# zer0int/OpenVision

Hardware: AMD Instinct MI355X
Metric: images/sec (node) ViT-L/14@224 fwd+InfoNCE (higher is better)
Workload: dtype bf16; 1 GPU; vit-large-patch14-224: image tower + text tower (T=80) + InfoNCE, per-GPU batch 256, formula weights, bf16 MFMA / fp32 accumulate; fp8_mask=0, global_batch=256, micro_batches=1, parallelism=dp1

## Files before the change

### include/ovhip.h

```cpp
#ifndef OVHIP_H
#define OVHIP_H

#include <stddef.h>
#include <stdint.h>

#ifdef __cplusplus
extern "C" {
#endif

#define OV_ABI_VERSION 2

typedef void* ov_stream_t;
typedef uint16_t ov_bf16;

enum ov_status {
    OV_OK = 0,
    OV_ERR_INVALID = -1,
    OV_ERR_UNSUPPORTED = -2,
    OV_ERR_WORKSPACE = -3,
    OV_ERR_NO_DEVICE = -4,
    OV_ERR_HIP = -1000
};

enum ov_dtype { OV_F32 = 0, OV_BF16 = 1 };
// ... 44 lines not shown
int ov_attention_lse(const ov_bf16* qkv, int64_t ld_qkv, ov_bf16* out, int64_t ld_out, float* lse, int B, int L, int H, int hd, float scale,
                     ov_stream_t stream);
int ov_attention_prefix(const ov_bf16* qkv, int64_t ld_qkv, ov_bf16* out, int64_t ld_out, int B, int L, int H, int hd, float scale,
                        int prefix, ov_stream_t stream);

int ov_im2col_patches(const void* image, int img_dtype, ov_bf16* out, int B, int S, int P, int Kpad,
                      ov_stream_t stream);

int ov_im2col_patches_keep(const void* image, int img_dtype, const int* keep, ov_bf16* out, int B, int S, int P, int K, int Kpad,
                           ov_stream_t stream);
int ov_patch_keep_inverse(const int* keep, int* inv, int B, int K, int G, int* err_flag, ov_stream_t stream);
int ov_patch_keep_assemble(const ov_bf16* y, int64_t ldy, const float* cls, const float* pos, const int* keep, float* x, int B, int K,
                           int G, int D, ov_stream_t stream);
int ov_patch_keep_assemble_backward(const float* dx, const int* inv, int B, int K, int G, int D, float* dpos, float* dcls, ov_bf16* dy,
                                    int64_t lddy, ov_stream_t stream);
int ov_col2im_patches_keep(const ov_bf16* dcols, int64_t ldc, const int* inv, void* dimg, int img_dtype, int B, int S, int P, int K,
                           ov_stream_t stream);

int ov_cls_rows(ov_bf16* x, int64_t ldx, const float* cls, const float* pos0, int B, int L, int D,
                ov_stream_t stream);

int ov_mean_pool(const ov_bf16* x, int64_t ldx, float* out, int B, int L, int D, int first,
                 ov_stream_t stream);

int ov_text_embed(const int64_t* tokens, const ov_bf16* table, const ov_bf16* pos, ov_bf16* x,
                  int64_t ldx, int B, int T, int D, int V, int* err_flag, ov_stream_t stream);

int ov_gather_rows(const ov_bf16* x, int64_t ldx, ov_bf16* out, int64_t ldo, int B, int L, int t, int D,
                   ov_stream_t stream);

int ov_convert(const void* src, int src_dtype, int64_t lds, void* dst, int dst_dtype, int64_t ldd,
               int64_t rows, int cols, ov_stream_t stream);

int ov_l2norm(const void* x, int x_dtype, int64_t ldx, float* y, int64_t ldy, int64_t rows, int E,
              ov_stream_t stream);

int ov_logits(const float* X, const float* Y, float* out, int64_t ldo, int n1, int n2, int E, float scale, const float* scale_dev,
              ov_stream_t stream);

int ov_attention_fp8out(const ov_bf16* qkv, int64_t ld_qkv, unsigned char* out8, int64_t ld_out, int B, int L, int H, int hd,
                        float scale, const float* out_amax, float* out_amax_next , ov_stream_t stream);

int ov_gemm_fp8(const unsigned char* A, int64_t lda, const unsigned char* W, int64_t ldw, const float* rowscale,
                const float* colscale, const float* bias, ov_bf16* C, int64_t ldc, int64_t M, int N, int K, int epilogue,
                const ov_bf16* R, int64_t ldr, ov_stream_t stream);

// ... 268 lines not shown
```

### openvision_amd/_lib.py

```python
from __future__ import annotations

import ctypes as C
import os
import threading

_PKG = os.path.dirname(os.path.abspath(__file__))
LIB_PATH = os.path.join(_PKG, "libovhip.so")
if os.environ.get("OVHIP_LIB"):
    LIB_PATH = os.path.join(_PKG, os.environ["OVHIP_LIB"]) if os.sep not in os.environ["OVHIP_LIB"] else os.environ["OVHIP_LIB"]

OV_F32, OV_BF16 = 0, 1
EPI_BIAS, EPI_GELU_ERF, EPI_GELU_TANH, EPI_RESIDUAL = 0, 1, 2, 3

c_void_p, c_int, c_int64, c_float, c_size_t = C.c_void_p, C.c_int, C.c_int64, C.c_float, C.c_size_t


class TowerCfg(C.Structure):
    _fields_ = [("width", c_int), ("layers", c_int), ("heads", c_int), ("mlp", c_int), ("mlp_pad", c_int),
                ("gelu_tanh", c_int), ("ln_eps", c_float)]


class BlockWeights(C.Structure):
    _fields_ = [(n, c_void_p) for n in ("ln1_w", "ln1_b", "qkv_w", "qkv_b", "out_w", "out_b", "ln2_w", "ln2_b",
                                        "fc_w", "fc_b", "proj_w", "proj_b", "qkv_colsum", "fc_colsum")]
# ... 54 lines not shown
    "ov_gemm_rowparts": (c_int, [c_void_p, c_int64, c_void_p, c_int64, c_void_p, c_void_p, c_int64, c_int64, c_int, c_int, c_void_p, c_int64,
                                 c_void_p, c_void_p]),
    "ov_attention": (c_int, [c_void_p, c_int64, c_void_p, c_int64, c_int, c_int, c_int, c_int, c_float, c_void_p]),
    "ov_attention_prefix": (c_int, [c_void_p, c_int64, c_void_p, c_int64, c_int, c_int, c_int, c_int, c_float, c_int, c_void_p]),
    "ov_attention_prefix_backward_workspace_bytes": (c_size_t, [c_int, c_int, c_int, c_int]),
    "ov_attention_prefix_backward": (c_int, [c_void_p, c_int64, c_void_p, c_int64, c_void_p, c_int64, c_void_p, c_int64, c_int, c_int, c_int,
                                             c_int, c_float, c_int, c_void_p, c_size_t, c_void_p]),
    "ov_softmax_xent_workspace_bytes": (c_size_t, [c_int64]),
    "ov_softmax_xent": (c_int, [c_void_p, c_int64, c_void_p, c_void_p, c_int64, c_int, c_void_p, c_void_p, c_void_p, c_size_t, c_void_p]),
    "ov_softmax_xent_backward": (c_int, [c_void_p, c_int64, c_void_p, c_void_p, c_void_p, c_void_p, c_void_p, c_int64, c_int64, c_int,
                                         c_void_p, c_size_t, c_void_p]),
    "ov_tower_set_prefix": (c_int, [c_void_p, c_int]),
    "ov_block_backward_prefix": (c_int, [c_void_p, c_void_p, c_void_p, c_void_p, c_void_p, c_void_p, c_void_p, c_int, c_int, c_int, c_void_p,
                                         c_size_t, c_void_p]),
    "ov_im2col_patches": (c_int, [c_void_p, c_int, c_void_p, c_int, c_int, c_int, c_int, c_void_p]),
    "ov_im2col_patches_keep": (c_int, [c_void_p, c_int, c_void_p, c_void_p, c_int, c_int, c_int, c_int, c_int, c_void_p]),
    "ov_patch_keep_inverse": (c_int, [c_void_p, c_void_p, c_int, c_int, c_int, c_void_p, c_void_p]),
    "ov_patch_keep_assemble": (c_int, [c_void_p, c_int64, c_void_p, c_void_p, c_void_p, c_void_p, c_int, c_int, c_int, c_int, c_void_p]),
    "ov_patch_keep_assemble_backward": (c_int, [c_void_p, c_void_p, c_int, c_int, c_int, c_int, c_void_p, c_void_p, c_void_p, c_int64,
                                                c_void_p]),
    "ov_col2im_patches_keep": (c_int, [c_void_p, c_int64, c_void_p, c_void_p, c_int, c_int, c_int, c_int, c_int, c_void_p]),
    "ov_cls_rows": (c_int, [c_void_p, c_int64, c_void_p, c_void_p, c_int, c_int, c_int, c_void_p]),
    "ov_mean_pool": (c_int, [c_void_p, c_int64, c_void_p, c_int, c_int, c_int, c_int, c_void_p]),
    "ov_text_embed": (c_int, [c_void_p, c_void_p, c_void_p, c_void_p, c_int64, c_int, c_int, c_int, c_int, c_void_p,
                              c_void_p]),
    "ov_gather_rows": (c_int, [c_void_p, c_int64, c_void_p, c_int64, c_int, c_int, c_int, c_int, c_void_p]),
    "ov_convert": (c_int, [c_void_p, c_int, c_int64, c_void_p, c_int, c_int64, c_int64, c_int, c_void_p]),
    "ov_l2norm": (c_int, [c_void_p, c_int, c_int64, c_void_p, c_int64, c_int64, c_int, c_void_p]),
    "ov_logits": (c_int, [c_void_p, c_void_p, c_void_p, c_int64, c_int, c_int, c_int, c_float, c_void_p, c_void_p]),
    "ov_preprocess_image": (c_int, [c_void_p, c_int, c_int, c_void_p, c_void_p, c_int, c_int, c_void_p, c_void_p, c_int, c_int, c_int,
                                    c_int, c_void_p, c_int, c_int, c_int, c_int, c_void_p, c_void_p, c_void_p, c_int, c_void_p]),
    "ov_class_mean_normalize": (c_int, [c_void_p, c_void_p, c_int, c_int, c_int, c_void_p]),
    "ov_topk": (c_int, [c_void_p, c_int64, c_int, c_int, c_int, c_int, c_void_p, c_void_p, c_void_p]),
    "ov_clip_loss_workspace_bytes": (c_size_t, [c_int, c_int]),
    "ov_clip_loss": (c_int, [c_void_p, c_void_p, c_void_p, c_void_p, c_int, c_int, c_int, c_void_p, c_int, c_void_p,
                             c_void_p, c_void_p, c_size_t, c_void_p]),
    "ov_clip_loss_backward_workspace_bytes": (c_size_t, [c_int, c_int]),
    "ov_clip_loss_multi_workspace_bytes": (c_size_t, [c_int, c_int, c_int]),
    "ov_clip_loss_multi": (c_int, [c_void_p, c_void_p, c_void_p, c_void_p, c_int64, c_int64, c_int, c_int, c_int, c_int, c_void_p, c_int,
                                   c_void_p, c_void_p, c_void_p, c_size_t, c_void_p]),
    "ov_clip_loss_multi_backward_workspace_bytes": (c_size_t, [c_int, c_int, c_int]),
    "ov_clip_loss_multi_backward": (c_int, [c_void_p, c_void_p, c_void_p, c_void_p, c_int64, c_int64, c_int, c_int, c_int, c_int, c_void_p,
                                            c_int, c_void_p, c_void_p, c_void_p, c_void_p, c_void_p, c_void_p, c_int64, c_int64, c_void_p,
                                            c_void_p, c_size_t, c_void_p]),
    "ov_siglip_loss_workspace_bytes": (c_size_t, [c_int, c_int]),
    "ov_siglip_loss": (c_int, [c_void_p, c_void_p, c_int, c_int, c_int, c_void_p, c_void_p, c_int, c_void_p, c_void_p, c_size_t,
# ... 130 lines not shown
```

### openvision_amd/csrc/embed.hip

```cpp
#include "common.h"

namespace {

template <bool IMG_F32>
__device__ __forceinline__ u32x4_t im2col_chunk(const void* __restrict__ img, int b, int py, int px, int ch, int S, int P) {
    const int PP = P * P, K = 3 * PP;
    float v[8];
#pragma unroll
    for (int e = 0; e < 8; ++e) {
        const int k = ch * 8 + e;
        float x = 0.f;
        if (k < K) {
            const int c = k / PP, rem = k - c * PP;
            const int ii = rem / P, jj = rem - ii * P;
            const int64_t src = (((int64_t)b * 3 + c) * S + (py * P + ii)) * S + (px * P + jj);
            x = IMG_F32 ? ((const float*)img)[src] : bf16_bits_to_f32(((const ov_bf16*)img)[src]);
        }
        v[e] = x;
    }
    return u32x4_t{pack_bf16x2(v[0], v[1]), pack_bf16x2(v[2], v[3]), pack_bf16x2(v[4], v[5]), pack_bf16x2(v[6], v[7])};
}

template <bool IMG_F32>
__global__ __launch_bounds__(256) void im2col_kernel(const void* __restrict__ img, ov_bf16* __restrict__ out,
// ... 180 lines not shown
        for (int t = first + wave; t < L; t += 4) {
            const u32x4_t w = *(const u32x4_t*)(p + (int64_t)t * ldx);
#pragma unroll
            for (int e = 0; e < 4; ++e) {
                acc[2 * e] += bf16lo_to_f32(w[e]);
                acc[2 * e + 1] += bf16hi_to_f32(w[e]);
            }
        }
    }
#pragma unroll
    for (int e = 0; e < 8; ++e) red[wave][lane][e] = acc[e];
    __syncthreads();
    if (wave == 0 && ch * 8 < D) {
        const float inv = 1.0f / (float)(L - first);
        float o[8];
#pragma unroll
        for (int e = 0; e < 8; ++e) o[e] = (red[0][lane][e] + red[1][lane][e] + red[2][lane][e] + red[3][lane][e]) * inv;
        float4* q = (float4*)(out + (int64_t)b * D + ch * 8);
        q[0] = make_float4(o[0], o[1], o[2], o[3]);
        q[1] = make_float4(o[4], o[5], o[6], o[7]);
    }
}

__global__ __launch_bounds__(256) void text_embed_kernel(const int64_t* __restrict__ tokens, const ov_bf16* __restrict__ table,
                                                         const ov_bf16* __restrict__ pos, ov_bf16* __restrict__ x, int64_t ldx,
                                                         int T, int D, int V, int* __restrict__ err, int64_t total) {
    const int cpr = D >> 3;
    for (int64_t i = (int64_t)blockIdx.x * blockDim.x + threadIdx.x; i < total; i += (int64_t)gridDim.x * blockDim.x) {
        const int64_t row = i / cpr;
        const int ch = (int)(i - row * cpr);
        const int t = (int)(row % T);
        int64_t id = tokens[row];
        if (id < 0 || id >= V) {
            if (err) *err = 1;
            id = id < 0 ? 0 : V - 1;
        }
        const u32x4_t a = *(const u32x4_t*)(table + id * D + ch * 8);
        const u32x4_t p = *(const u32x4_t*)(pos + (int64_t)t * D + ch * 8);
        u32x4_t o;
#pragma unroll
        for (int e = 0; e < 4; ++e)
            o[e] = pack_bf16x2(bf16lo_to_f32(a[e]) + bf16lo_to_f32(p[e]), bf16hi_to_f32(a[e]) + bf16hi_to_f32(p[e]));
        *(u32x4_t*)(x + row * ldx + ch * 8) = o;
    }
}

// ... 91 lines not shown
    OV_LAUNCH_CHECK();
    return OV_OK;
}

extern "C" int ov_cls_rows(ov_bf16* x, int64_t ldx, const float* cls, const float* pos0, int B, int L, int D,
                           ov_stream_t stream) {
    if (!x || !cls || !pos0 || B <= 0 || L <= 0 || D <= 0 || ldx < D) return OV_ERR_INVALID;
    hipLaunchKernelGGL(cls_rows_kernel, dim3(grid_for((int64_t)B * D, 256)), dim3(256), 0, (hipStream_t)stream, x, ldx, cls,
                       pos0, B, L, D);
    OV_LAUNCH_CHECK();
    return OV_OK;
}

extern "C" int ov_mean_pool(const ov_bf16* x, int64_t ldx, float* out, int B, int L, int D, int first,
                            ov_stream_t stream) {
    if (!x || !out || B <= 0 || L <= 0 || D <= 0 || first < 0 || first >= L) return OV_ERR_INVALID;
    if (D % 8 || ldx % 8 || ldx < D || (((uintptr_t)x | (uintptr_t)out) & 15)) return OV_ERR_INVALID;
    hipLaunchKernelGGL(mean_pool_kernel, dim3((unsigned)B, (unsigned)((D / 8 + 63) / 64)), dim3(256), 0, (hipStream_t)stream, x,
                       ldx, out, L, D, first);
    OV_LAUNCH_CHECK();
    return OV_OK;
}

extern "C" int ov_text_embed(const int64_t* tokens, const ov_bf16* table, const ov_bf16* pos, ov_bf16* x, int64_t ldx,
                             int B, int T, int D, int V, int* err_flag, ov_stream_t stream) {
    if (!tokens || !table || !pos || !x || B <= 0 || T <= 0 || D <= 0 || V <= 0) return OV_ERR_INVALID;
    if (D % 8 || ldx % 8 || ldx < D || (((uintptr_t)table | (uintptr_t)pos | (uintptr_t)x) & 15)) return OV_ERR_INVALID;
    const int64_t total = (int64_t)B * T * (D / 8);
    hipLaunchKernelGGL(text_embed_kernel, dim3(grid_for(total, 256)), dim3(256), 0, (hipStream_t)stream, tokens, table, pos, x,
                       ldx, T, D, V, err_flag, total);
    OV_LAUNCH_CHECK();
    return OV_OK;
}

extern "C" int ov_gather_rows(const ov_bf16* x, int64_t ldx, ov_bf16* out, int64_t ldo, int B, int L, int t, int D,
                              ov_stream_t stream) {
    if (!x || !out || B <= 0 || L <= 0 || t < 0 || t >= L || D <= 0) return OV_ERR_INVALID;
    if (D % 8 || ldx % 8 || ldo % 8 || ldx < D || ldo < D || (((uintptr_t)x | (uintptr_t)out) & 15)) return OV_ERR_INVALID;
    hipLaunchKernelGGL(gather_rows_kernel, dim3(grid_for((int64_t)B * (D / 8), 256)), dim3(256), 0, (hipStream_t)stream, x, ldx,
                       out, ldo, B, L, t, D);
    OV_LAUNCH_CHECK();
    return OV_OK;
}

extern "C" int ov_convert(const void* src, int src_dtype, int64_t lds, void* dst, int dst_dtype, int64_t ldd, int64_t rows,
                          int cols, ov_stream_t stream) {
// ... 91 lines not shown
```

### openvision_amd/csrc/tower.hip

```cpp
#include "common.h"
#include <new>
#include <vector>
#include <mutex>
#include <stdlib.h>

struct TailCtx {
    hipStream_t stream = nullptr;
    hipEvent_t fork = nullptr, join = nullptr;
    int state = 0;
    int device = -1;
    std::mutex mu;
};

struct ov_tower {
    mutable TailCtx tail;
    ov_tower_cfg cfg;
    ov_block_weights* blocks;
    unsigned char* set;
    ov_block_fp8* fp8;
    unsigned char* set8;
    float* h_amax;
    int h_mode;
    unsigned char* mask8;
    int prefix;
// ... 252 lines not shown
    return OV_OK;
}

extern "C" int ov_tower_set_prefix(ov_tower* t, int prefix) {
    if (!t || prefix < -1) return OV_ERR_INVALID;
    t->prefix = prefix;
    return OV_OK;
}

extern "C" size_t ov_tower_workspace_bytes(const ov_tower* t, int B, int L) {
    if (!t || B <= 0 || L <= 0) return 0;
    const size_t M = (size_t)B * L;
    const int D = t->cfg.width;
    size_t n = align_up(M * D * 2, 256) + align_up(M * (size_t)big_pitch(t->cfg) * 2, 256) + align_up(M * 8, 256) +
               align_up(M * (size_t)(D / 32) * 8, 256);
    if (tower_fp8(t)) n += align_up(M * (size_t)max_i(D, t->cfg.mlp_pad), 256) + align_up(M * 4, 256);
    return n;
}

namespace {
struct BlockPart { ov_bf16 *x, *h, *big; float *stats, *parts; unsigned char* q8; float* qs; int B; ov_stream_t stream; bool prof; };
struct Fp8Scales { float *h_amax, *a_amax, *h_next, *a_next; int h_mode; };

int run_block(const ov_tower_cfg& c, const ov_block_weights& w, const ov_block_fp8* q, int mask, const Fp8Scales& sc, const BlockPart& p,
              bool parts_in, int L, int prefix) {
    const int D = c.width, H = c.heads, hd = D / H, F = c.mlp_pad, B = p.B;
    const int64_t M = (int64_t)B * L;
    const int ldb = big_pitch(c);
    const float scale = 1.0f / sqrtf((float)hd);
    const int gelu = c.gelu_tanh ? OV_EPI_BIAS_GELU_TANH : OV_EPI_BIAS_GELU_ERF;
    const int fc_cls = c.gelu_tanh ? OV_PROF_GEMM_FC_TANH : OV_PROF_GEMM_FC;
    const bool fold = w.qkv_colsum != nullptr && w.fc_colsum != nullptr;
    const bool rp = fold && p.parts != nullptr;
    const bool f_qkv = mask & OV_FP8_QKV, f_out = mask & OV_FP8_OUT, f_fc = mask & OV_FP8_FC, f_proj = mask & OV_FP8_PROJ;
    ov_bf16 *x = p.x, *h = p.h, *big = p.big;
    float *stats = p.stats, *parts = p.parts, *qs = p.qs;
    unsigned char* q8 = p.q8;
    ov_stream_t stream = p.stream;
    int rc;
#define OV_STEP(cls, call)                                             \
    do {                                                               \
        if (p.prof) { ProfScope ps__(cls, stream, M); rc = (call); }   \
        else rc = (call);                                              \
        if (rc) return rc;                                             \
    } while (0)
    if (f_qkv) {
        OV_STEP(OV_PROF_LN, ov_layernorm_quant_fp8(x, D, w.ln1_w, w.ln1_b, q8, D, qs, M, D, c.ln_eps, stream));
        OV_STEP(OV_PROF_GEMM_QKV, ov_gemm_fp8(q8, D, q->qkv_w8, D, qs, q->qkv_s, q->qkv_b, big, ldb, M, 3 * D, D, OV_EPI_BIAS, nullptr, 0, stream));
    } else if (fold) {
        if (rp && parts_in) OV_STEP(OV_PROF_LN, ov_rowstats_finalize(parts, stats, M, D, c.ln_eps, stream));
        else OV_STEP(OV_PROF_LN, ov_rowstats(x, D, stats, M, D, c.ln_eps, stream));
        OV_STEP(OV_PROF_GEMM_QKV, ov_gemm_ln(x, D, w.qkv_w, D, w.qkv_b, w.qkv_colsum, stats, big, ldb, M, 3 * D, D, OV_EPI_BIAS, stream));
    } else {
        OV_STEP(OV_PROF_LN, ov_layernorm(x, OV_BF16, D, w.ln1_w, w.ln1_b, h, OV_BF16, D, M, D, c.ln_eps, stream));
        OV_STEP(OV_PROF_GEMM_QKV, ov_gemm(h, D, w.qkv_w, D, w.qkv_b, big, ldb, M, 3 * D, D, OV_EPI_BIAS, nullptr, 0, 0, 0, 0, stream));
    }
    if (f_out && sc.h_mode >= 2 && hd == 64) {
        OV_STEP(OV_PROF_ATTN, ov_attention_fp8out(big, ldb, q8, D, B, L, H, hd, scale, sc.a_amax, sc.a_next, stream));
        OV_STEP(OV_PROF_GEMM_OUT, ov_gemm_fp8_static(q8, D, q->out_w8, D, nullptr, sc.a_amax, q->out_s, w.out_b, x, D, nullptr, nullptr, M, D, D,
                                                     OV_EPI_BIAS_RESIDUAL, x, D, stream));
    } else {
        if (prefix >= 0) OV_STEP(OV_PROF_ATTN, ov_attention_prefix(big, ldb, h, D, B, L, H, hd, scale, prefix, stream));
        else OV_STEP(OV_PROF_ATTN, ov_attention(big, ldb, h, D, B, L, H, hd, scale, stream));
        if (f_out) {
            OV_STEP(OV_PROF_LN, ov_quant_rows_fp8(h, D, q8, D, qs, M, D, sc.h_mode == 1 ? sc.a_amax : nullptr, stream));
            OV_STEP(OV_PROF_GEMM_OUT, ov_gemm_fp8(q8, D, q->out_w8, D, qs, q->out_s, w.out_b, x, D, M, D, D, OV_EPI_BIAS_RESIDUAL, x, D, stream));
        } else if (rp) {
            OV_STEP(OV_PROF_GEMM_OUT, ov_gemm_rowparts(h, D, w.out_w, D, w.out_b, x, D, M, D, D, x, D, parts, stream));
        } else {
            OV_STEP(OV_PROF_GEMM_OUT, ov_gemm(h, D, w.out_w, D, w.out_b, x, D, M, D, D, OV_EPI_BIAS_RESIDUAL, x, D, 0, 0, 0, stream));
        }
    }
    if (f_fc) {
        OV_STEP(OV_PROF_LN, ov_layernorm_quant_fp8(x, D, w.ln2_w, w.ln2_b, q8, D, qs, M, D, c.ln_eps, stream));
    } else if (fold) {
        if (rp) OV_STEP(OV_PROF_LN, ov_rowstats_finalize(parts, stats, M, D, c.ln_eps, stream));
        else OV_STEP(OV_PROF_LN, ov_rowstats(x, D, stats, M, D, c.ln_eps, stream));
    } else {
        OV_STEP(OV_PROF_LN, ov_layernorm(x, OV_BF16, D, w.ln2_w, w.ln2_b, h, OV_BF16, D, M, D, c.ln_eps, stream));
    }
    if (f_fc && f_proj && sc.h_mode >= 2) {
        unsigned char* h8 = (unsigned char*)big;
        OV_STEP(fc_cls, ov_gemm_fp8_static(q8, D, q->fc_w8, D, qs, nullptr, q->fc_s, q->fc_b, h8, F, sc.h_amax, sc.h_next, M, F, D, gelu, nullptr, 0,
                                           stream));
        OV_STEP(OV_PROF_GEMM_PROJ, ov_gemm_fp8_static(h8, F, q->proj_w8, F, nullptr, sc.h_amax, q->proj_s, w.proj_b, x, D, nullptr, nullptr, M, D, F,
                                                      OV_EPI_BIAS_RESIDUAL, x, D, stream));
    } else {
        if (f_fc) OV_STEP(fc_cls, ov_gemm_fp8(q8, D, q->fc_w8, D, qs, q->fc_s, q->fc_b, big, ldb, M, F, D, gelu, nullptr, 0, stream));
        else if (fold) OV_STEP(fc_cls, ov_gemm_ln(x, D, w.fc_w, D, w.fc_b, w.fc_colsum, stats, big, ldb, M, F, D, gelu, stream));
        else OV_STEP(fc_cls, ov_gemm(h, D, w.fc_w, D, w.fc_b, big, ldb, M, F, D, gelu, nullptr, 0, 0, 0, 0, stream));
        if (f_proj) {
            OV_STEP(OV_PROF_LN, ov_quant_rows_fp8(big, ldb, q8, F, qs, M, F, (sc.h_mode == 1 && f_fc) ? sc.h_amax : nullptr, stream));
            OV_STEP(OV_PROF_GEMM_PROJ, ov_gemm_fp8(q8, F, q->proj_w8, F, qs, q->proj_s, w.proj_b, x, D, M, D, F, OV_EPI_BIAS_RESIDUAL, x, D, stream));
        } else if (rp) {
            OV_STEP(OV_PROF_GEMM_PROJ, ov_gemm_rowparts(big, ldb, w.proj_w, F, w.proj_b, x, D, M, D, F, x, D, parts, stream));
        } else {
            OV_STEP(OV_PROF_GEMM_PROJ, ov_gemm(big, ldb, w.proj_w, F, w.proj_b, x, D, M, D, F, OV_EPI_BIAS_RESIDUAL, x, D, 0, 0, 0, stream));
        }
    }
#undef OV_STEP
    return OV_OK;
}

TailCtx* tail_ctx(const ov_tower* t) {
    TailCtx& tc = t->tail;
    std::lock_guard<std::mutex> lk(tc.mu);
    if (tc.state == 0) {
        const char* e = getenv("OVHIP_NO_TAIL_SPLIT");
        if (e && e[0] == '1') { tc.state = -1; return nullptr; }
        tc.device = ov_current_device();
        if (hipStreamCreateWithFlags(&tc.stream, hipStreamNonBlocking) == hipSuccess &&
            hipEventCreateWithFlags(&tc.fork, hipEventDisableTiming) == hipSuccess &&
            hipEventCreateWithFlags(&tc.join, hipEventDisableTiming) == hipSuccess)
            tc.state = 1;
        else
            tc.state = -1;
    }
    return tc.state == 1 && tc.device == ov_current_device() ? &tc : nullptr;
}

int tail_images(int B, int L) {
    const int64_t T = ((int64_t)B * L + 255) / 256;
    const int r = (int)(T % 64);
    if (T <= 64 || r == 0 || r > 8) return 0;
    const int64_t target = T - r;
    int Bm = (int)((target * 256) / L);
    while (Bm > 0 && ((int64_t)Bm * L + 255) / 256 > target) --Bm;
    const int tail = B - Bm;
    if (Bm <= 0 || tail <= 0 || tail > B / 8) return 0;
    return tail;
}
}

extern "C" int ov_tower_forward(const ov_tower* t, ov_bf16* x, int B, int L, void* workspace, size_t workspace_bytes,
                                ov_stream_t stream) {
    if (!t || !x || !workspace || B <= 0 || L <= 0) return OV_ERR_INVALID;
    if (workspace_bytes < ov_tower_workspace_bytes(t, B, L)) return OV_ERR_WORKSPACE;
    if (((uintptr_t)x | (uintptr_t)workspace) & 15) return OV_ERR_INVALID;
    const ov_tower_cfg& c = t->cfg;
    const int D = c.width;
    const int64_t M = (int64_t)B * L;
    const int ldb = big_pitch(c);
    ov_bf16* h = (ov_bf16*)workspace;
    ov_bf16* big = (ov_bf16*)((char*)workspace + align_up((size_t)M * D * 2, 256));
    float* stats = (float*)((char*)big + align_up((size_t)M * ldb * 2, 256));
    for (int i = 0; i < c.layers; ++i)
        if (!t->set[i]) return OV_ERR_INVALID;

    int nt = tail_images(B, L);
    TailCtx* tc = nt > 0 ? tail_ctx(t) : nullptr;
    if (!tc) nt = 0;
    const int Bm = B - nt;
    hipStream_t main_st = (hipStream_t)stream;
    std::unique_lock<std::mutex> tail_lock;
    if (nt > 0) {
        tail_lock = std::unique_lock<std::mutex>(tc->mu);
        hipError_t e = hipEventRecord(tc->fork, main_st);
        if (e == hipSuccess) e = hipStreamWaitEvent(tc->stream, tc->fork, 0);
        if (e != hipSuccess) return OV_ERR_HIP - (int)e;
    }
    const int64_t off = (int64_t)Bm * L;
    const bool fp8 = tower_fp8(t);
    if (t->prefix >= 0 && fp8) return OV_ERR_UNSUPPORTED;
    if (t->prefix > L) return OV_ERR_INVALID;
    int rc = OV_OK;
    if (fp8 && t->h_amax && t->h_mode == 2)
        rc = ov_amax_roll(t->h_amax, t->h_amax + 2 * c.layers, 2 * c.layers, stream);
    const int G = D / 32;
    float* parts = use_rowparts() && !fp8 ? (float*)((char*)workspace + ov_tower_workspace_bytes(t, B, L) - align_up((size_t)M * G * 8, 256)) : nullptr;
    const int qw = D > c.mlp_pad ? D : c.mlp_pad;
    unsigned char* q8 = (unsigned char*)stats + align_up((size_t)M * 8, 256);
    float* qs = (float*)(q8 + align_up((size_t)M * qw, 256));
    const BlockPart main_part = {x, h, big, stats, parts, q8, qs, Bm, stream, true};
    const BlockPart tail_part = {x + off * D, h + off * D, big + off * ldb, stats + 2 * off, parts ? parts + 2 * off * G : nullptr,
                                 q8 + off * qw, qs + off, nt, (ov_stream_t)(nt > 0 ? tc->stream : nullptr), false};
    for (int i = 0; i < c.layers && rc == OV_OK; ++i) {
        Fp8Scales sc = {nullptr, nullptr, nullptr, nullptr, 0};
        if (t->h_amax) sc = {t->h_amax + i, t->h_amax + c.layers + i, t->h_amax + 2 * c.layers + i, t->h_amax + 3 * c.layers + i, t->h_mode};
        const ov_block_fp8* q = fp8 ? &t->fp8[i] : nullptr;
        const int mask = fp8 ? t->mask8[i] : 0;
        rc = run_block(c, t->blocks[i], q, mask, sc, main_part, i > 0, L, t->prefix);
        if (rc == OV_OK && nt > 0) rc = run_block(c, t->blocks[i], q, mask, sc, tail_part, i > 0, L, t->prefix);
    }
    if (nt > 0) {
        hipError_t e = hipEventRecord(tc->join, tc->stream);
        if (e == hipSuccess) e = hipStreamWaitEvent(main_st, tc->join, 0);
        if (e != hipSuccess && rc == OV_OK) rc = OV_ERR_HIP - (int)e;
    }
    return rc;
}

int block_grad_pairs(const ov_block_grads* g);
int block_backward_partial(const ov_tower_cfg* cfg, const ov_block_weights* w, const ov_bf16* x, const ov_block_saved* s, const ov_bf16* dy,
                           ov_bf16* dx, const ov_block_grads* g, int prefix, int B, int L, void* workspace, size_t workspace_bytes,
                           ov_stream_t stream);
size_t block_backward_input_workspace_bytes(const ov_tower_cfg* cfg, int B, int L);
int block_backward_input(const ov_tower_cfg* cfg, const ov_block_weights* w, const ov_bf16* x, const ov_block_saved* s, const ov_bf16* dy,
                         ov_bf16* dx, int prefix, int B, int L, void* workspace, ov_stream_t stream);

static inline size_t saved_per_token(const ov_tower_cfg& c) { return (size_t)8 * c.width + 2 * (size_t)c.mlp_pad; }
static inline size_t saved_lse_elems(const ov_tower_cfg& c, int B, int L) {
    return ((size_t)2 * B * c.heads * ((L + 31) / 32 * 32) + 7) / 8 * 8;
}
static inline size_t saved_per_layer(const ov_tower_cfg& c, int B, int L) { return (size_t)B * L * saved_per_token(c) + saved_lse_elems(c, B, L); }
extern "C" size_t ov_tower_saved_bytes(const ov_tower* t, int B, int L) {
    if (!t || B <= 0 || L <= 0) return 0;
    return (size_t)t->cfg.layers * saved_per_layer(t->cfg, B, L) * sizeof(ov_bf16);
}

namespace {
struct Slot { ov_bf16 *x, *qkv, *o, *x1, *n1, *n2, *pre, *act; float* lse; };
inline Slot slot_at(const ov_tower_cfg& c, ov_bf16* sx, ov_bf16* rest, int64_t M) {
// ... 239 lines not shown
extern "C" int ov_vision_embed(const ov_tower* t, const ov_vision_head* h, const void* image, int img_dtype, int B,
                               ov_bf16* x, void* workspace, size_t workspace_bytes, ov_stream_t stream) {
    if (!t || !h || !image || !x || !workspace || B <= 0) return OV_ERR_INVALID;
    const int g = h->image_size / h->patch_size, L = g * g + 1, D = t->cfg.width;
    const size_t need = (size_t)B * g * g * h->kpad * 2;
    if (workspace_bytes < need) return OV_ERR_WORKSPACE;
    if (h->kpad % 64 || h->kpad < 3 * h->patch_size * h->patch_size) return OV_ERR_INVALID;
    ov_bf16* patches = (ov_bf16*)workspace;
    int rc;
    if ((rc = ov_im2col_patches(image, img_dtype, patches, B, h->image_size, h->patch_size, h->kpad, stream))) return rc;
    if ((rc = ov_gemm(patches, h->kpad, h->conv_w, h->kpad, nullptr, x, D, (int64_t)B * g * g, D, h->kpad,
                      OV_EPI_BIAS_RESIDUAL, h->pos, D, g * g, g * g, 1, stream)))
        return rc;
    return ov_cls_rows(x, D, h->cls, h->pos_f32, B, L, D, stream);
}

extern "C" int ov_vision_head_forward(const ov_tower* t, const ov_vision_head* h, const ov_bf16* x, int B, float* features,
                                      int normalize, void* workspace, size_t workspace_bytes, ov_stream_t stream) {
    if (!t || !h || !x || !features || !workspace || B <= 0 || h->patch_size <= 0) return OV_ERR_INVALID;
    const int g = h->image_size / h->patch_size;
    return ov_vision_head_forward_tokens(t, h, x, B, g * g + 1, features, normalize, workspace, workspace_bytes, stream);
}

extern "C" int ov_vision_head_forward_tokens(const ov_tower* t, const ov_vision_head* h, const ov_bf16* x, int B, int L, float* features,
                                             int normalize, void* workspace, size_t workspace_bytes, ov_stream_t stream) {
    if (!t || !h || !x || !features || !workspace || B <= 0 || L < 2) return OV_ERR_INVALID;
    const int D = t->cfg.width, E = h->embed_dim, EP = h->embed_pad;
    if (EP % 8 || EP < E) return OV_ERR_INVALID;
    if (!h->final_ln_after_pool) return OV_ERR_UNSUPPORTED;
    const size_t o_pooled = 0, o_ln = align_up((size_t)B * D * 4, 256), o_feat = o_ln + align_up((size_t)B * D * 2, 256);
    if (workspace_bytes < o_feat + (size_t)B * EP * 2) return OV_ERR_WORKSPACE;
    float* pooled = (float*)((char*)workspace + o_pooled);
    ov_bf16* ln = (ov_bf16*)((char*)workspace + o_ln);
    ov_bf16* feat = (ov_bf16*)((char*)workspace + o_feat);
    int rc;
    if (h->pool_avg) {
        if ((rc = ov_mean_pool(x, D, pooled, B, L, D, 1, stream))) return rc;
        if ((rc = ov_layernorm(pooled, OV_F32, D, h->ln_post_w, h->ln_post_b, ln, OV_BF16, D, B, D, t->cfg.ln_eps, stream))) return rc;
    } else {
        if ((rc = ov_layernorm(x, OV_BF16, (int64_t)L * D, h->ln_post_w, h->ln_post_b, ln, OV_BF16, D, B, D, t->cfg.ln_eps, stream)))
            return rc;
    }
    if ((rc = ov_gemm(ln, D, h->proj_t, D, nullptr, feat, EP, B, EP, D, OV_EPI_BIAS, nullptr, 0, 0, 0, 0, stream))) return rc;
    if (normalize) return ov_l2norm(feat, OV_BF16, EP, features, E, B, E, stream);
    return ov_convert(feat, OV_BF16, EP, features, OV_F32, E, B, E, stream);
}

extern "C" int ov_encode_image(const ov_tower* t, const ov_vision_head* h, const void* image, int img_dtype, int B,
                               float* features, int normalize, void* workspace, size_t workspace_bytes, ov_stream_t stream) {
    if (!t || !h || !image || !features || !workspace || B <= 0) return OV_ERR_INVALID;
    const VisionWs w = vision_ws(t, h, B);
    if (workspace_bytes < w.total) return OV_ERR_WORKSPACE;
    const int g = h->image_size / h->patch_size, L = g * g + 1;
    char* ws = (char*)workspace;
    ov_bf16* x = (ov_bf16*)(ws + w.x);
    const size_t tower_bytes = ov_tower_workspace_bytes(t, B, L);
    int rc;
    if ((size_t)B * g * g * h->kpad * 2 > tower_bytes) return OV_ERR_WORKSPACE;
    if ((rc = ov_vision_embed(t, h, image, img_dtype, B, x, ws + w.tower, tower_bytes, stream))) return rc;
    if ((rc = ov_tower_forward(t, x, B, L, ws + w.tower, tower_bytes, stream))) return rc;
    return ov_vision_head_forward(t, h, x, B, features, normalize, ws + w.pooled, w.total - w.pooled, stream);
}

int ov_im2col_patches_keep_pos(const void* image, int img_dtype, const int* keep, ov_bf16* out, int B, int S, int P, int K, int Kpad,
                               const ov_bf16* pos, ov_bf16* posk, int D, int* err_flag, ov_stream_t stream);

extern "C" size_t ov_vision_keep_workspace_bytes(const ov_tower* t, const ov_vision_head* h, int B, int K) {
    if (!t || !h || B <= 0 || h->patch_size <= 0) return 0;
    const int g = h->image_size / h->patch_size;
    if (K < 1 || K > g * g) return 0;
    return vision_keep_ws(t, h, B, K).total;
}

extern "C" int ov_vision_embed_keep(const ov_tower* t, const ov_vision_head* h, const void* image, int img_dtype, const int* keep, int B,
                                    int K, ov_bf16* x, int* err_flag, void* workspace, size_t workspace_bytes, ov_stream_t stream) {
    if (!t || !h || !image || !keep || !x || !workspace || B <= 0 || h->patch_size <= 0) return OV_ERR_INVALID;
    const int g = h->image_size / h->patch_size, D = t->cfg.width;
    if (K < 1 || K > g * g) return OV_ERR_INVALID;
    if (h->kpad % 64 || h->kpad < 3 * h->patch_size * h->patch_size) return OV_ERR_INVALID;
    if (workspace_bytes < keep_embed_bytes(t, h, B, K)) return OV_ERR_WORKSPACE;
    ov_bf16* patches = (ov_bf16*)workspace;
    ov_bf16* posk = (ov_bf16*)((char*)workspace + align_up((size_t)B * K * h->kpad * 2, 256));
    int rc;
    if ((rc = ov_im2col_patches_keep_pos(image, img_dtype, keep, patches, B, h->image_size, h->patch_size, K, h->kpad, h->pos, posk, D,
                                         err_flag, stream)))
        return rc;
    if ((rc = ov_gemm(patches, h->kpad, h->conv_w, h->kpad, nullptr, x, D, (int64_t)B * K, D, h->kpad, OV_EPI_BIAS_RESIDUAL, posk, D, K, 0,
                      0, stream)))
        return rc;
    return ov_cls_rows(x, D, h->cls, h->pos_f32, B, K + 1, D, stream);
}

extern "C" int ov_encode_image_keep(const ov_tower* t, const ov_vision_head* h, const void* image, int img_dtype, const int* keep, int B,
                                    int K, float* features, int normalize, int* err_flag, void* workspace, size_t workspace_bytes,
                                    ov_stream_t stream) {
    if (!t || !h || !image || !keep || !features || !workspace || B <= 0 || h->patch_size <= 0) return OV_ERR_INVALID;
    const int g = h->image_size / h->patch_size;
    if (K < 1 || K > g * g) return OV_ERR_INVALID;
    const VisionWs w = vision_keep_ws(t, h, B, K);
    if (workspace_bytes < w.total) return OV_ERR_WORKSPACE;
    const int L = K + 1;
    char* ws = (char*)workspace;
    ov_bf16* x = (ov_bf16*)(ws + w.x);
    int rc;
    if ((rc = ov_vision_embed_keep(t, h, image, img_dtype, keep, B, K, x, err_flag, ws + w.tower, w.pooled - w.tower, stream))) return rc;
    if ((rc = ov_tower_forward(t, x, B, L, ws + w.tower, w.pooled - w.tower, stream))) return rc;
    return ov_vision_head_forward_tokens(t, h, x, B, L, features, normalize, ws + w.pooled, w.total - w.pooled, stream);
}

extern "C" size_t ov_text_workspace_bytes(const ov_tower* t, const ov_text_head* h, int B) {
    if (!t || !h || B <= 0) return 0;
    return text_ws(t, h, B).total;
}

extern "C" int ov_encode_text(const ov_tower* t, const ov_text_head* h, const int64_t* tokens, int B, float* features,
                              int normalize, int* err_flag, void* workspace, size_t workspace_bytes, ov_stream_t stream) {
    if (!t || !h || !tokens || !features || !workspace || B <= 0) return OV_ERR_INVALID;
    const TextWs w = text_ws(t, h, B);
    if (workspace_bytes < w.total) return OV_ERR_WORKSPACE;
    const int T = h->context_length, D = t->cfg.width, E = h->embed_dim, EP = (E + 7) / 8 * 8;
    char* ws = (char*)workspace;
    ov_bf16* x = (ov_bf16*)(ws + w.x);
    ov_bf16* last = (ov_bf16*)(ws + w.last);
    ov_bf16* ln = (ov_bf16*)(ws + w.lnrow);
    ov_bf16* feat = (ov_bf16*)(ws + w.feat);
    int rc;
    if ((rc = ov_text_embed(tokens, h->token_embedding, h->pos, x, D, B, T, D, h->vocab_size, err_flag, stream))) return rc;
    if ((rc = ov_tower_forward(t, x, B, T, ws + w.tower, ov_tower_workspace_bytes(t, B, T), stream))) return rc;
    if ((rc = ov_gather_rows(x, D, last, D, B, T, h->pool_last ? T - 1 : 0, D, stream))) return rc;
    if ((rc = ov_layernorm(last, OV_BF16, D, h->ln_final_w, h->ln_final_b, ln, OV_BF16, D, B, D, t->cfg.ln_eps, stream))) return rc;
    if ((rc = ov_gemm(ln, D, h->proj_t, D, nullptr, feat, EP, B, EP, D, OV_EPI_BIAS, nullptr, 0, 0, 0, 0, stream))) return rc;
    if (normalize) return ov_l2norm(feat, OV_BF16, EP, features, E, B, E, stream);
    return ov_convert(feat, OV_BF16, EP, features, OV_F32, E, B, E, stream);
}
```

Baseline: 5616 images/sec.

## Skip unused last-block work using pooling linearity and last-token-only tail

For the vision tower with average pooling, the last block's MLP projection runs on the mean-pooled hidden activations instead of every token, since a linear projection commutes with the mean. This is done with a new small fp32 MFMA pooled-linear kernel that adds onto the pooled residual. For the text tower, only the pooled row goes through the last block's out-projection, LN, FC and projection after attention. This drops most of the final block's GEMM work. It changes rounding slightly (fp32 mean before the projection) and can be turned off with OVHIP_LAST_BLOCK_FULL=1.

After: 5679 images/sec (median of 6 runs). 1.1% higher.

```diff
diff --git a/include/ovhip.h b/include/ovhip.h
--- a/include/ovhip.h
+++ b/include/ovhip.h
@@ -90,6 +90,10 @@
 
 int ov_mean_pool(const ov_bf16* x, int64_t ldx, float* out, int B, int L, int D, int first,
                  ov_stream_t stream);
+
+size_t ov_mlp_out_pooled_workspace_bytes(int B, int F);
+int ov_mlp_out_pooled(const ov_bf16* x1, int64_t ldx, const ov_bf16* hid, int64_t ldh, const ov_bf16* W, int64_t ldw, const float* bias,
+                      float* out, int B, int L, int D, int F, int first, void* workspace, size_t workspace_bytes, ov_stream_t stream);
 
 int ov_text_embed(const int64_t* tokens, const ov_bf16* table, const ov_bf16* pos, ov_bf16* x,
                   int64_t ldx, int B, int T, int D, int V, int* err_flag, ov_stream_t stream);
diff --git a/openvision_amd/_lib.py b/openvision_amd/_lib.py
--- a/openvision_amd/_lib.py
+++ b/openvision_amd/_lib.py
@@ -100,6 +100,9 @@
     "ov_col2im_patches_keep": (c_int, [c_void_p, c_int64, c_void_p, c_void_p, c_int, c_int, c_int, c_int, c_int, c_void_p]),
     "ov_cls_rows": (c_int, [c_void_p, c_int64, c_void_p, c_void_p, c_int, c_int, c_int, c_void_p]),
     "ov_mean_pool": (c_int, [c_void_p, c_int64, c_void_p, c_int, c_int, c_int, c_int, c_void_p]),
+    "ov_mlp_out_pooled_workspace_bytes": (c_size_t, [c_int, c_int]),
+    "ov_mlp_out_pooled": (c_int, [c_void_p, c_int64, c_void_p, c_int64, c_void_p, c_int64, c_void_p, c_void_p, c_int, c_int, c_int, c_int,
+                                  c_int, c_void_p, c_size_t, c_void_p]),
     "ov_text_embed": (c_int, [c_void_p, c_void_p, c_void_p, c_void_p, c_int64, c_int, c_int, c_int, c_int, c_void_p,
                               c_void_p]),
     "ov_gather_rows": (c_int, [c_void_p, c_int64, c_void_p, c_int64, c_int, c_int, c_int, c_int, c_void_p]),
diff --git a/openvision_amd/csrc/embed.hip b/openvision_amd/csrc/embed.hip
--- a/openvision_amd/csrc/embed.hip
+++ b/openvision_amd/csrc/embed.hip
@@ -226,6 +226,46 @@
     }
 }
 
+__global__ __launch_bounds__(256) void pooled_linear_kernel(const float* __restrict__ A, const ov_bf16* __restrict__ W, int64_t ldw,
+                                                            const float* __restrict__ bias, float* __restrict__ out, int B, int N,
+                                                            int K) {
+    __shared__ float red[4][16][64];
+    const int lane = threadIdx.x & 63, wave = threadIdx.x >> 6;
+    const int j = lane & 31, half = lane >> 5;
+    const int i0 = blockIdx.y * 32, j0 = blockIdx.x * 32;
+    const int ai = (i0 + j) < B ? (i0 + j) : B - 1;
+    const int wj = (j0 + j) < N ? (j0 + j) : N - 1;
+    const int kq = K >> 2;
+    const float* ap = A + (int64_t)ai * K + wave * kq + 4 * half;
+    const ov_bf16* wp = W + (int64_t)wj * ldw + wave * kq + 4 * half;
+    f32x16_t acc;
+#pragma unroll
+    for (int i = 0; i < 16; ++i) acc[i] = 0.f;
+#pragma unroll 4
+    for (int k0 = 0; k0 < kq; k0 += 8) {
+        const u32x2_t wv = *(const u32x2_t*)(wp + k0);
+        const float4 av = *(const float4*)(ap + k0);
+        acc = __builtin_amdgcn_mfma_f32_32x32x2f32(bf16lo_to_f32(wv[0]), av.x, acc, 0, 0, 0);
+        acc = __builtin_amdgcn_mfma_f32_32x32x2f32(bf16hi_to_f32(wv[0]), av.y, acc, 0, 0, 0);
+        acc = __builtin_amdgcn_mfma_f32_32x32x2f32(bf16lo_to_f32(wv[1]), av.z, acc, 0, 0, 0);
+        acc = __builtin_amdgcn_mfma_f32_32x32x2f32(bf16hi_to_f32(wv[1]), av.w, acc, 0, 0, 0);
+    }
+#pragma unroll
+    for (int i = 0; i < 16; ++i) red[wave][i][lane] = acc[i];
+    __syncthreads();
+    if (wave == 0 && i0 + j < B) {
+#pragma unroll
+        for (int i = 0; i < 16; ++i) {
+            const int col = j0 + (i & 3) + 8 * (i >> 2) + 4 * half;
+            if (col < N) {
+                const float s = ((red[0][i][lane] + red[1][i][lane]) + red[2][i][lane]) + red[3][i][lane];
+                float* o = out + (int64_t)(i0 + j) * N + col;
+                *o = *o + (s + bias[col]);
+            }
+        }
+    }
+}
+
 __global__ __launch_bounds__(256) void text_embed_kernel(const int64_t* __restrict__ tokens, const ov_bf16* __restrict__ table,
                                                          const ov_bf16* __restrict__ pos, ov_bf16* __restrict__ x, int64_t ldx,
                                                          int T, int D, int V, int* __restrict__ err, int64_t total) {
@@ -363,6 +403,26 @@
     return OV_OK;
 }
 
+extern "C" size_t ov_mlp_out_pooled_workspace_bytes(int B, int F) {
+    return B > 0 && F > 0 ? (size_t)B * F * 4 : 0;
+}
+
+extern "C" int ov_mlp_out_pooled(const ov_bf16* x1, int64_t ldx, const ov_bf16* hid, int64_t ldh, const ov_bf16* W, int64_t ldw,
+                                 const float* bias, float* out, int B, int L, int D, int F, int first, void* workspace,
+                                 size_t workspace_bytes, ov_stream_t stream) {
+    if (!x1 || !hid || !W || !bias || !out || !workspace || B <= 0 || L <= 0 || D <= 0 || F <= 0) return OV_ERR_INVALID;
+    if (F % 32 || ldw % 8 || ldw < F || (((uintptr_t)W | (uintptr_t)workspace | (uintptr_t)bias) & 15)) return OV_ERR_INVALID;
+    if (workspace_bytes < ov_mlp_out_pooled_workspace_bytes(B, F)) return OV_ERR_WORKSPACE;
+    float* mean_h = (float*)workspace;
+    int rc;
+    if ((rc = ov_mean_pool(x1, ldx, out, B, L, D, first, stream))) return rc;
+    if ((rc = ov_mean_pool(hid, ldh, mean_h, B, L, F, first, stream))) return rc;
+    hipLaunchKernelGGL(pooled_linear_kernel, dim3((unsigned)((D + 31) / 32), (unsigned)((B + 31) / 32)), dim3(256), 0,
+                       (hipStream_t)stream, mean_h, W, ldw, bias, out, B, D, F);
+    OV_LAUNCH_CHECK();
+    return OV_OK;
+}
+
 extern "C" int ov_text_embed(const int64_t* tokens, const ov_bf16* table, const ov_bf16* pos, ov_bf16* x, int64_t ldx,
                              int B, int T, int D, int V, int* err_flag, ov_stream_t stream) {
     if (!tokens || !table || !pos || !x || B <= 0 || T <= 0 || D <= 0 || V <= 0) return OV_ERR_INVALID;
diff --git a/openvision_amd/csrc/tower.hip b/openvision_amd/csrc/tower.hip
--- a/openvision_amd/csrc/tower.hip
+++ b/openvision_amd/csrc/tower.hip
@@ -298,8 +298,9 @@
 struct BlockPart { ov_bf16 *x, *h, *big; float *stats, *parts; unsigned char* q8; float* qs; int B; ov_stream_t stream; bool prof; };
 struct Fp8Scales { float *h_amax, *a_amax, *h_next, *a_next; int h_mode; };
 
+enum BlockStop { BLOCK_FULL = 0, BLOCK_TO_ATTN = 1, BLOCK_TO_FC = 2 };
 int run_block(const ov_tower_cfg& c, const ov_block_weights& w, const ov_block_fp8* q, int mask, const Fp8Scales& sc, const BlockPart& p,
-              bool parts_in, int L, int prefix) {
+              bool parts_in, int L, int prefix, int stop = BLOCK_FULL) {
     const int D = c.width, H = c.heads, hd = D / H, F = c.mlp_pad, B = p.B;
     const int64_t M = (int64_t)B * L;
     const int ldb = big_pitch(c);
@@ -338,6 +339,7 @@
     } else {
         if (prefix >= 0) OV_STEP(OV_PROF_ATTN, ov_attention_prefix(big, ldb, h, D, B, L, H, hd, scale, prefix, stream));
         else OV_STEP(OV_PROF_ATTN, ov_attention(big, ldb, h, D, B, L, H, hd, scale, stream));
+        if (stop == BLOCK_TO_ATTN) return OV_OK;
         if (f_out) {
             OV_STEP(OV_PROF_LN, ov_quant_rows_fp8(h, D, q8, D, qs, M, D, sc.h_mode == 1 ? sc.a_amax : nullptr, stream));
             OV_STEP(OV_PROF_GEMM_OUT, ov_gemm_fp8(q8, D, q->out_w8, D, qs, q->out_s, w.out_b, x, D, M, D, D, OV_EPI_BIAS_RESIDUAL, x, D, stream));
@@ -365,6 +367,7 @@
         if (f_fc) OV_STEP(fc_cls, ov_gemm_fp8(q8, D, q->fc_w8, D, qs, q->fc_s, q->fc_b, big, ldb, M, F, D, gelu, nullptr, 0, stream));
         else if (fold) OV_STEP(fc_cls, ov_gemm_ln(x, D, w.fc_w, D, w.fc_b, w.fc_colsum, stats, big, ldb, M, F, D, gelu, stream));
         else OV_STEP(fc_cls, ov_gemm(h, D, w.fc_w, D, w.fc_b, big, ldb, M, F, D, gelu, nullptr, 0, 0, 0, 0, stream));
+        if (stop == BLOCK_TO_FC) return OV_OK;
         if (f_proj) {
             OV_STEP(OV_PROF_LN, ov_quant_rows_fp8(big, ldb, q8, F, qs, M, F, (sc.h_mode == 1 && f_fc) ? sc.h_amax : nullptr, stream));
             OV_STEP(OV_PROF_GEMM_PROJ, ov_gemm_fp8(q8, F, q->proj_w8, F, qs, q->proj_s, w.proj_b, x, D, M, D, F, OV_EPI_BIAS_RESIDUAL, x, D, stream));
@@ -408,8 +411,8 @@
 }
 }
 
-extern "C" int ov_tower_forward(const ov_tower* t, ov_bf16* x, int B, int L, void* workspace, size_t workspace_bytes,
-                                ov_stream_t stream) {
+static int tower_walk(const ov_tower* t, ov_bf16* x, int B, int L, void* workspace, size_t workspace_bytes, ov_stream_t stream,
+                      int last_stop) {
     if (!t || !x || !workspace || B <= 0 || L <= 0) return OV_ERR_INVALID;
     if (workspace_bytes < ov_tower_workspace_bytes(t, B, L)) return OV_ERR_WORKSPACE;
     if (((uintptr_t)x | (uintptr_t)workspace) & 15) return OV_ERR_INVALID;
@@ -438,6 +441,7 @@
     const int64_t off = (int64_t)Bm * L;
     const bool fp8 = tower_fp8(t);
     if (t->prefix >= 0 && fp8) return OV_ERR_UNSUPPORTED;
+    if (last_stop != BLOCK_FULL && fp8) return OV_ERR_UNSUPPORTED;
     if (t->prefix > L) return OV_ERR_INVALID;
     int rc = OV_OK;
     if (fp8 && t->h_amax && t->h_mode == 2)
@@ -455,8 +459,9 @@
         if (t->h_amax) sc = {t->h_amax + i, t->h_amax + c.layers + i, t->h_amax + 2 * c.layers + i, t->h_amax + 3 * c.layers + i, t->h_mode};
         const ov_block_fp8* q = fp8 ? &t->fp8[i] : nullptr;
         const int mask = fp8 ? t->mask8[i] : 0;
-        rc = run_block(c, t->blocks[i], q, mask, sc, main_part, i > 0, L, t->prefix);
-        if (rc == OV_OK && nt > 0) rc = run_block(c, t->blocks[i], q, mask, sc, tail_part, i > 0, L, t->prefix);
+        const int stop = i == c.layers - 1 ? last_stop : BLOCK_FULL;
+        rc = run_block(c, t->blocks[i], q, mask, sc, main_part, i > 0, L, t->prefix, stop);
+        if (rc == OV_OK && nt > 0) rc = run_block(c, t->blocks[i], q, mask, sc, tail_part, i > 0, L, t->prefix, stop);
     }
     if (nt > 0) {
         hipError_t e = hipEventRecord(tc->join, tc->stream);
@@ -464,6 +469,17 @@
         if (e != hipSuccess && rc == OV_OK) rc = OV_ERR_HIP - (int)e;
     }
     return rc;
+}
+
+extern "C" int ov_tower_forward(const ov_tower* t, ov_bf16* x, int B, int L, void* workspace, size_t workspace_bytes,
+                                ov_stream_t stream) {
+    return tower_walk(t, x, B, L, workspace, workspace_bytes, stream, BLOCK_FULL);
+}
+
+static inline bool last_block_full() {
+    static int v = -1;
+    if (v < 0) { const char* e = getenv("OVHIP_LAST_BLOCK_FULL"); v = (e && e[0] == '1') ? 1 : 0; }
+    return v != 0;
 }
 
 int block_grad_pairs(const ov_block_grads* g);
@@ -749,28 +765,70 @@
     return ov_vision_head_forward_tokens(t, h, x, B, g * g + 1, features, normalize, workspace, workspace_bytes, stream);
 }
 
-extern "C" int ov_vision_head_forward_tokens(const ov_tower* t, const ov_vision_head* h, const ov_bf16* x, int B, int L, float* features,
-                                             int normalize, void* workspace, size_t workspace_bytes, ov_stream_t stream) {
-    if (!t || !h || !x || !features || !workspace || B <= 0 || L < 2) return OV_ERR_INVALID;
+namespace {
+struct HeadBufs { float* pooled; ov_bf16 *ln, *feat; };
+int head_bufs(const ov_tower* t, const ov_vision_head* h, int B, void* workspace, size_t workspace_bytes, HeadBufs* hb) {
     const int D = t->cfg.width, E = h->embed_dim, EP = h->embed_pad;
     if (EP % 8 || EP < E) return OV_ERR_INVALID;
     if (!h->final_ln_after_pool) return OV_ERR_UNSUPPORTED;
     const size_t o_pooled = 0, o_ln = align_up((size_t)B * D * 4, 256), o_feat = o_ln + align_up((size_t)B * D * 2, 256);
     if (workspace_bytes < o_feat + (size_t)B * EP * 2) return OV_ERR_WORKSPACE;
-    float* pooled = (float*)((char*)workspace + o_pooled);
-    ov_bf16* ln = (ov_bf16*)((char*)workspace + o_ln);
-    ov_bf16* feat = (ov_bf16*)((char*)workspace + o_feat);
+    hb->pooled = (float*)((char*)workspace + o_pooled);
+    hb->ln = (ov_bf16*)((char*)workspace + o_ln);
+    hb->feat = (ov_bf16*)((char*)workspace + o_feat);
+    return OV_OK;
+}
+int head_finish(const ov_tower* t, const ov_vision_head* h, const HeadBufs& hb, bool pooled, int B, float* features, int normalize,
+                ov_stream_t stream) {
+    const int D = t->cfg.width, E = h->embed_dim, EP = h->embed_pad;
     int rc;
+    if (pooled && (rc = ov_layernorm(hb.pooled, OV_F32, D, h->ln_post_w, h->ln_post_b, hb.ln, OV_BF16, D, B, D, t->cfg.ln_eps, stream)))
+        return rc;
+    if ((rc = ov_gemm(hb.ln, D, h->proj_t, D, nullptr, hb.feat, EP, B, EP, D, OV_EPI_BIAS, nullptr, 0, 0, 0, 0, stream))) return rc;
+    if (normalize) return ov_l2norm(hb.feat, OV_BF16, EP, features, E, B, E, stream);
+    return ov_convert(hb.feat, OV_BF16, EP, features, OV_F32, E, B, E, stream);
+}
+}
+
+extern "C" int ov_vision_head_forward_tokens(const ov_tower* t, const ov_vision_head* h, const ov_bf16* x, int B, int L, float* features,
+                                             int normalize, void* workspace, size_t workspace_bytes, ov_stream_t stream) {
+    if (!t || !h || !x || !features || !workspace || B <= 0 || L < 2) return OV_ERR_INVALID;
+    const int D = t->cfg.width;
+    HeadBufs hb;
+    int rc;
+    if ((rc = head_bufs(t, h, B, workspace, workspace_bytes, &hb))) return rc;
     if (h->pool_avg) {
-        if ((rc = ov_mean_pool(x, D, pooled, B, L, D, 1, stream))) return rc;
-        if ((rc = ov_layernorm(pooled, OV_F32, D, h->ln_post_w, h->ln_post_b, ln, OV_BF16, D, B, D, t->cfg.ln_eps, stream))) return rc;
+        if ((rc = ov_mean_pool(x, D, hb.pooled, B, L, D, 1, stream))) return rc;
     } else {
-        if ((rc = ov_layernorm(x, OV_BF16, (int64_t)L * D, h->ln_post_w, h->ln_post_b, ln, OV_BF16, D, B, D, t->cfg.ln_eps, stream)))
+        if ((rc = ov_layernorm(x, OV_BF16, (int64_t)L * D, h->ln_post_w, h->ln_post_b, hb.ln, OV_BF16, D, B, D, t->cfg.ln_eps, stream)))
             return rc;
     }
-    if ((rc = ov_gemm(ln, D, h->proj_t, D, nullptr, feat, EP, B, EP, D, OV_EPI_BIAS, nullptr, 0, 0, 0, 0, stream))) return rc;
-    if (normalize) return ov_l2norm(feat, OV_BF16, EP, features, E, B, E, stream);
-    return ov_convert(feat, OV_BF16, EP, features, OV_F32, E, B, E, stream);
+    return head_finish(t, h, hb, h->pool_avg != 0, B, features, normalize, stream);
+}
+
+static int blocks_and_head(const ov_tower* t, const ov_vision_head* h, ov_bf16* x, int B, int L, char* tower_ws, size_t tower_bytes,
+                           char* head_ws, size_t head_bytes, float* features, int normalize, ov_stream_t stream) {
+    const ov_tower_cfg& c = t->cfg;
+    const int D = c.width, F = c.mlp_pad;
+    const size_t h_bytes = align_up((size_t)B * L * D * 2, 256);
+    const bool pooled_tail = !last_block_full() && h->pool_avg && h->final_ln_after_pool && L >= 2 && !tower_fp8(t) && F % 32 == 0 &&
+                             ov_mlp_out_pooled_workspace_bytes(B, F) <= h_bytes;
+    int rc;
+    if (!pooled_tail) {
+        if ((rc = ov_tower_forward(t, x, B, L, tower_ws, tower_bytes, stream))) return rc;
+        return ov_vision_head_forward_tokens(t, h, x, B, L, features, normalize, head_ws, head_bytes, stream);
+    }
+    HeadBufs hb;
+    if ((rc = head_bufs(t, h, B, head_ws, head_bytes, &hb))) return rc;
+    if ((rc = tower_walk(t, x, B, L, tower_ws, tower_bytes, stream, BLOCK_TO_FC))) return rc;
+    const ov_block_weights& lw = t->blocks[c.layers - 1];
+    const ov_bf16* hidden = (const ov_bf16*)(tower_ws + h_bytes);
+    {
+        ProfScope ps(OV_PROF_GEMM_PROJ, stream, B);
+        rc = ov_mlp_out_pooled(x, D, hidden, big_pitch(c), lw.proj_w, F, lw.proj_b, hb.pooled, B, L, D, F, 1, tower_ws, h_bytes, stream);
+    }
+    if (rc) return rc;
+    return head_finish(t, h, hb, true, B, features, normalize, stream);
 }
 
 extern "C" int ov_encode_image(const ov_tower* t, const ov_vision_head* h, const void* image, int img_dtype, int B,
@@ -785,8 +843,7 @@
     int rc;
     if ((size_t)B * g * g * h->kpad * 2 > tower_bytes) return OV_ERR_WORKSPACE;
     if ((rc = ov_vision_embed(t, h, image, img_dtype, B, x, ws + w.tower, tower_bytes, stream))) return rc;
-    if ((rc = ov_tower_forward(t, x, B, L, ws + w.tower, tower_bytes, stream))) return rc;
-    return ov_vision_head_forward(t, h, x, B, features, normalize, ws + w.pooled, w.total - w.pooled, stream);
+    return blocks_and_head(t, h, x, B, L, ws + w.tower, tower_bytes, ws + w.pooled, w.total - w.pooled, features, normalize, stream);
 }
 
 int ov_im2col_patches_keep_pos(const void* image, int img_dtype, const int* keep, ov_bf16* out, int B, int S, int P, int K, int Kpad,
@@ -831,6 +888,8 @@
     ov_bf16* x = (ov_bf16*)(ws + w.x);
     int rc;
     if ((rc = ov_vision_embed_keep(t, h, image, img_dtype, keep, B, K, x, err_flag, ws + w.tower, w.pooled - w.tower, stream))) return rc;
+    if (K == g * g)
+        return blocks_and_head(t, h, x, B, L, ws + w.tower, w.pooled - w.tower, ws + w.pooled, w.total - w.pooled, features, normalize, stream);
     if ((rc = ov_tower_forward(t, x, B, L, ws + w.tower, w.pooled - w.tower, stream))) return rc;
     return ov_vision_head_forward_tokens(t, h, x, B, L, features, normalize, ws + w.pooled, w.total - w.pooled, stream);
 }
@@ -853,8 +912,42 @@
     ov_bf16* feat = (ov_bf16*)(ws + w.feat);
     int rc;
     if ((rc = ov_text_embed(tokens, h->token_embedding, h->pos, x, D, B, T, D, h->vocab_size, err_flag, stream))) return rc;
-    if ((rc = ov_tower_forward(t, x, B, T, ws + w.tower, ov_tower_workspace_bytes(t, B, T), stream))) return rc;
-    if ((rc = ov_gather_rows(x, D, last, D, B, T, h->pool_last ? T - 1 : 0, D, stream))) return rc;
+    const size_t tower_bytes = ov_tower_workspace_bytes(t, B, T);
+    const int row = h->pool_last ? T - 1 : 0;
+    const ov_tower_cfg& c = t->cfg;
+    const int F = c.mlp_pad;
+    const size_t o_n = align_up((size_t)B * D * 2, 256), o_hid = 2 * o_n, o_stats = o_hid + align_up((size_t)B * F * 2, 256);
+    const size_t h_bytes = align_up((size_t)B * T * D * 2, 256), big_bytes = align_up((size_t)B * T * big_pitch(c) * 2, 256);
+    if (last_block_full() || tower_fp8(t) || o_stats + (size_t)B * 8 > big_bytes) {
+        if ((rc = ov_tower_forward(t, x, B, T, ws + w.tower, tower_bytes, stream))) return rc;
+        if ((rc = ov_gather_rows(x, D, last, D, B, T, row, D, stream))) return rc;
+    } else {
+        if ((rc = tower_walk(t, x, B, T, ws + w.tower, tower_bytes, stream, BLOCK_TO_ATTN))) return rc;
+        const ov_block_weights& lw = t->blocks[c.layers - 1];
+        const ov_bf16* attn = (const ov_bf16*)(ws + w.tower);
+        char* big = ws + w.tower + h_bytes;
+        ov_bf16 *a = (ov_bf16*)big, *n = (ov_bf16*)(big + o_n), *hid = (ov_bf16*)(big + o_hid);
+        float* stats = (float*)(big + o_stats);
+        const int gelu = c.gelu_tanh ? OV_EPI_BIAS_GELU_TANH : OV_EPI_BIAS_GELU_ERF;
+#define OV_TAIL_STEP(cls, call)                                    \
+        do {                                                       \
+            { ProfScope ps__(cls, stream, B); rc = (call); }       \
+            if (rc) return rc;                                     \
+        } while (0)
+        const int fc_cls = c.gelu_tanh ? OV_PROF_GEMM_FC_TANH : OV_PROF_GEMM_FC;
+        if ((rc = ov_gather_rows(attn, D, a, D, B, T, row, D, stream))) return rc;
+        if ((rc = ov_gather_rows(x, D, last, D, B, T, row, D, stream))) return rc;
+        OV_TAIL_STEP(OV_PROF_GEMM_OUT, ov_gemm(a, D, lw.out_w, D, lw.out_b, last, D, B, D, D, OV_EPI_BIAS_RESIDUAL, last, D, 0, 0, 0, stream));
+        if (lw.fc_colsum) {
+            OV_TAIL_STEP(OV_PROF_LN, ov_rowstats(last, D, stats, B, D, c.ln_eps, stream));
+            OV_TAIL_STEP(fc_cls, ov_gemm_ln(last, D, lw.fc_w, D, lw.fc_b, lw.fc_colsum, stats, hid, F, B, F, D, gelu, stream));
+        } else {
+            OV_TAIL_STEP(OV_PROF_LN, ov_layernorm(last, OV_BF16, D, lw.ln2_w, lw.ln2_b, n, OV_BF16, D, B, D, c.ln_eps, stream));
+            OV_TAIL_STEP(fc_cls, ov_gemm(n, D, lw.fc_w, D, lw.fc_b, hid, F, B, F, D, gelu, nullptr, 0, 0, 0, 0, stream));
+        }
+        OV_TAIL_STEP(OV_PROF_GEMM_PROJ, ov_gemm(hid, F, lw.proj_w, F, lw.proj_b, last, D, B, D, F, OV_EPI_BIAS_RESIDUAL, last, D, 0, 0, 0, stream));
+#undef OV_TAIL_STEP
+    }
     if ((rc = ov_layernorm(last, OV_BF16, D, h->ln_final_w, h->ln_final_b, ln, OV_BF16, D, B, D, t->cfg.ln_eps, stream))) return rc;
     if ((rc = ov_gemm(ln, D, h->proj_t, D, nullptr, feat, EP, B, EP, D, OV_EPI_BIAS, nullptr, 0, 0, 0, 0, stream))) return rc;
     if (normalize) return ov_l2norm(feat, OV_BF16, EP, features, E, B, E, stream);
```
